# yuw444/fastF

Measured on AMD Instinct MI355X. Metric: BAM records/sec -> deduped UMI matrix; achieved HBM GB/s vs roofline, higher is better.
Workload: dtype u64

## Files before the change

### fastf_amd/csrc/umi_engine.hip

```cpp
#include "umi_kernels.hpp"
#include "sweep_kernels.hpp"

#include <algorithm>
#include <cstdarg>
#include <cstdio>
#include <cstdlib>
#include <cstring>
#include <initializer_list>
#include <mutex>
#include <new>
#include <stdexcept>
#include <chrono>
#include <string>
#include <thread>
#include <utility>
#include <vector>

extern "C" {
#include "fastf_amd.h"
#include "host_io.h"
#include "mt_jump.h"
}

using namespace fastf;
// ... 132 lines not shown
    for (size_t o = 0; o < bytes; o += HostBounce::BYTES) {
        const size_t n = std::min(bytes - o, HostBounce::BYTES);
        memcpy(g_bounce.p, (const char*)h_src + o, n);
        HIP_OK(hipMemcpyAsync((char*)d_dst + o, g_bounce.p, n, hipMemcpyHostToDevice, s));
        HIP_OK(hipStreamSynchronize(s));
    }
    return 0;
}

struct KernelTimer {
    std::vector<std::pair<hipEvent_t, hipEvent_t>> ev;
    size_t used = 0;
};

enum { AN_CAP_HITS, AN_GENE_SUMMARY, AN_GENE_MOMENTS, AN_NBR_GRAM, AN_LABEL_VOTES, AN_MARKER_AUC, AN_FAMILIES };
struct AnalysisState {
    bool attr[AN_FAMILIES] = {};
    DevBuf d_nbr;
    DevBuf d_coex;
};

enum { T_K1A, T_SCATTER, T_K3, T_COUNT, T_K1B, T_GATHER, T_TIMERS };

struct fastf_multi;
struct fastf_engine {
    fastf_multi* multi = nullptr;
    int device = 0;
    hipStream_t s_compute = nullptr, s_copy = nullptr, s_mt = nullptr;
    hipEvent_t ev_mt = nullptr;
    KeyLayout L{};
    u32 cell_bits = 0, feat_bits = 0, n_cells = 0, n_features = 0;
    u64 threshold = 0;
    u32 n_shards = 1, shard_rank = 0;
    DevBuf tab_cells, tab_feats;
    Table cells{}, feats{};
    DevBuf img_cells, img_genes;
    DevBuf d_cell_filter; MissFilter cell_filter{nullptr, 0};
    CellLds lds_cells{}; GeneLds lds_genes{};
    bool cell16 = false;
    bool use_lds_cells = false, use_lds_genes = false; u32 genes_blocks_per_cu = 1, cells_blocks_per_cu = 1;
    fastf_mt_t mt{};
    u32 mt_seed0 = 0; u64 mt_skip0 = 0;
    u64 mt_hits = 0;
    u64 mt_abs0 = 0;
    bool mt_live = false;
    DevBuf d_ring; u64 ring_len = 0;
    u32 ring_carry = 0;
    DevBuf d_dbits;
    DevBuf d_mtwords;
    bool mtwords_kept = false; u32 mtwords_seed = 0; u64 mtwords_skip = 0, mtwords_n = 0;
    AnalysisState an;
    DevBuf d_mt; bool mt_on_device = false;
    u32 mt_dev_idx = MT_N;
    bool mt_par_ready = false;
    DevBuf d_mtsub, d_mtpoly, d_mtseat, d_mtseq;
    u64 draws_up = 0;
    u64 draws_valid = 0;
    u64 batch_cap = 0;
    struct Slot {
        void* h_stage = nullptr;
        void* h_draws = nullptr;
        DevBuf d_stage;
        hipEvent_t ev_copy = nullptr, ev_done = nullptr;
        u64* h_small = nullptr;
        bool busy = false; u64 n = 0; bool external = false;
    } slot[2];
    int cur = 0;
    const u32* cur_umi_ext = nullptr;
    u64 inflight_records = 0;
    u64 key_cap = 0;
    DevBuf d_keys, d_tmp;
    DevBuf d_small;
    u64* h_small = nullptr;
    DevBuf d_feature, d_cell, d_count, d_ukeys, d_ncopy;
    u32* h_coo = nullptr; u64 h_coo_cap = 0, h_nnz = 0;
    bool h_coo_pinned = false; u32 h_coo_uses = 0;
    u32* lent_rows = nullptr; u64 lent_cap = 0;
    u32* rows_at = nullptr; u64 rows_stride = 0;
    std::vector<u32> h_ufeature, h_ucell, h_uumi, h_ncopy;
    std::vector<uint8_t> h_unonnull;
    u64 total_records = 0, hits_so_far = 0, keys_so_far = 0;
    u64 c_sampled = 0, c_valid = 0;
    bool finished = false; int sorted_in_tmp = 0; u64 n_sorted = 0;
    u32 skip_bits = 0;
    bool fully_sorted = false;
    DevBuf d_cellidx, d_tilecnt, d_tilebase, d_binbase, d_cnt;
    DevBuf d_halfhits;
    DevBuf d_segkeys;
    DevBuf d_segcount, d_segprefix, d_tileseg;
    u32 giant_parity = 0;
    u32 seg_n = 0; u64 seg_stride = 0;
    DevBuf d_rgn_phys, d_rgn_hist, d_rgn_blk;
    u32 rgn_hist_n = 0, rgn_hist_shift = 0;
    bool stream_mode = false, store_regions = false;
    bool stream_single = false, stream_sharded = false, stream_off = false;
    bool narrow = false, genes_one_family = false;
    u64 slots_used = 0, slot_cap = 0; u32 rgn_n = 0, rgn_cap = 0;
    DevBuf d_scanblk;
    u32 grid_cus = 256; int tile_grid_cap = 0; u32 k3_per_cu = 4;
    DevBuf d_rg_feature, d_rg_cell, d_rg_count, d_rg_ukeys, d_spanrows, d_spanbase, d_giant;
    u32 rg_n = 0; bool rg_umi = false;
    bool wide = false, long_umi = false; u32 group_bits = 0;
    u32 sub_bits = 0, row_split = 0;
    bool finish_queued = false;
    DevBuf d_vals, d_vtmp;
    bool timing = false;
// ... 183 lines not shown
    const u32 words = (u32)((range + 31) / 32), rank_pad = (words + 1u) & ~1u;
    size_t bytes = (((size_t)words * 4 + (size_t)rank_pad * 2 + best_n * 2) + 15) & ~(size_t)15;
    const size_t direct_bytes = ((size_t)range * 2 + 15) & ~(size_t)15;
    const bool direct = direct_bytes <= bytes + bytes / 8 && !getenv("FASTF_GENES_NO_DIRECT");
    if (direct) bytes = direct_bytes;
    {
        const char* mk = getenv("FASTF_GENES_LDS_MAX_KB");
        if (bytes > (size_t)(mk ? atoi(mk) : 152) * 1024) return 0;
    }
    std::vector<u32> img(bytes / 4 + 4, 0u);
    if (direct) {
        unsigned short* tab = reinterpret_cast<unsigned short*>(img.data());
        for (u32 i = 0; i < n; ++i) if ((keys[i] >> 44) == best) tab[(keys[i] & VM) - vmin] = (unsigned short)(i + 1);
    }
    u32* bitmap = img.data();
    unsigned short* rank = reinterpret_cast<unsigned short*>(img.data() + words);
    unsigned short* perm = rank + rank_pad;
    if (!direct) {
        std::vector<std::pair<u64, u32>> vals; vals.reserve(best_n);
        for (u32 i = 0; i < n; ++i) if ((keys[i] >> 44) == best) vals.push_back({(keys[i] & VM) - vmin, i + 1});
        std::sort(vals.begin(), vals.end());
        for (size_t r = 0; r < vals.size(); ++r) { bitmap[vals[r].first >> 5] |= 1u << (vals[r].first & 31); perm[r] = (unsigned short)vals[r].second; }
        u32 acc = 0;
        for (u32 w = 0; w < words; ++w) { rank[w] = (unsigned short)acc; acc += (u32)__builtin_popcount(bitmap[w]); }
    }
    if (e->img_genes.ensure(bytes)) return 1;
    if (copy_h2d(e->img_genes.p, img.data(), bytes)) return 1;
    e->lds_genes.image = (const u32*)e->img_genes.p; e->lds_genes.words = words; e->lds_genes.n_perm = (u32)best_n;
    e->lds_genes.family = (u32)best; e->lds_genes.vmin = vmin; e->lds_genes.range = range; e->lds_genes.bytes = (u32)bytes; e->lds_genes.direct = direct ? 1u : 0u;
    {
        for (const void* f : {(const void*)filter_pack_kernel<true, false>, (const void*)filter_pack_kernel<true, true>})
            if (hipFuncSetAttribute(f, hipFuncAttributeMaxDynamicSharedMemorySize, (int)bytes) != hipSuccess) return 0;
        for (u32 i = 0; i < N_STREAM_KERNELS; ++i)
            if (hipFuncSetAttribute((const void*)stream_kernel(i), hipFuncAttributeMaxDynamicSharedMemorySize, (int)bytes) != hipSuccess) return 0;
    }
    const size_t per_block = bytes + 1024;
    e->genes_blocks_per_cu = (u32)std::max<size_t>(1, std::min<size_t>(3, (160 * 1024) / per_block));
    e->use_lds_genes = true;
    e->genes_one_family = best_n == n;
    return 0;
}
template <size_t... I> static StreamKernel stream_kernel_of(u32 i, std::index_sequence<I...>) {
    static const StreamKernel k[] = {filter_pack_stream_kernel<(I & 4) != 0, (I & 2) != 0, (I & 1) != 0, (I >> 3) >= 1, (I >> 3) == 2>...};
    return k[i];
}
static StreamKernel stream_kernel(u32 i) { return stream_kernel_of(i, std::make_index_sequence<N_STREAM_KERNELS>{}); }

static void decide_stream_k1b(fastf_engine* e) {
    const bool can = e->use_lds_genes && !e->wide;
    e->stream_single = can && e->n_shards == 1;
    e->stream_sharded = can && e->n_shards > 1 && e->n_shards <= (u32)MAX_SHARDS;
    e->stream_off = getenv("FASTF_NO_STREAM_K1B") != nullptr;
}

extern "C" int fastf_engine_create(const fastf_engine_config_t* cfg, fastf_engine_t** out) FASTF_TRY {
    if (!cfg || !out) return set_err("null argument");
    *out = nullptr;
    const char* pf_ = getenv("FASTF_PROFILE");
    const bool lap_on = pf_ && pf_[0] == '2';
    const auto t_0 = std::chrono::steady_clock::now();
    auto lap = [&](const char* what) { if (lap_on) fprintf(stderr, "[engine create] %s at %.1f ms\n", what, std::chrono::duration<double, std::milli>(std::chrono::steady_clock::now() - t_0).count()); };
    int ndev = 0;
    hipError_t he = hipGetDeviceCount(&ndev);
    lap("device count");
    if (he != hipSuccess || ndev == 0)
        return set_err("no HIP device available (%s): the engine has no CPU fallback", hipGetErrorString(he));
    if (cfg->umi_max_bases < 1 || cfg->umi_max_bases > 32) return set_err("umi_max_bases must be 1..32");
    if (cfg->n_devices > 1 || (cfg->n_devices == 1 && getenv("FASTF_FORCE_MULTI"))) {
        fastf_engine* me = new fastf_engine();
        if (multi_create(cfg, me)) { multi_destroy(me); delete me; return 1; }
        *out = me;
        return 0;
    }
    if (cfg->device < 0 || cfg->device >= ndev) return set_err("device %d out of range (have %d)", cfg->device, ndev);
    if (cfg->n_shards < 1 || cfg->n_shards > 8 || cfg->shard_rank >= cfg->n_shards) return set_err("bad shard config");
    HIP_OK(hipSetDevice(cfg->device));
    { hipDeviceProp_t pr; if (hipGetDeviceProperties(&pr, cfg->device) == hipSuccess && pr.multiProcessorCount > 0) g_cu_count = (u32)pr.multiProcessorCount; }
    lap("device set, properties");

    fastf_engine* e = new fastf_engine();
    e->device = cfg->device;
    {
        e->grid_cus = g_cu_count;
        const char* gc = getenv("FASTF_GRID_CUS");
        if (gc) e->grid_cus = (u32)std::min<long>(std::max<long>(atol(gc), 1), (long)g_cu_count);
        const char* tc = getenv("FASTF_TILE_GRID_CAP");
        e->tile_grid_cap = tc ? std::max(atoi(tc), 8) : 0;
        const char* kc = getenv("FASTF_K3_PER_CU");
        e->k3_per_cu = kc ? (u32)std::max(atoi(kc), 1) : 4u;
    }
    e->n_cells = cfg->n_cells; e->n_features = cfg->n_features;
    e->cell16 = cfg->n_cells <= 65535u && !getenv("FASTF_CELL_SCRATCH_32");
    e->cell_bits = bits_for(cfg->n_cells);
    e->feat_bits = bits_for(cfg->n_features);
    e->L.umi_bits = 2 * cfg->umi_max_bases;
    e->L.umi_max_bytes = (cfg->umi_max_bases + 3) / 4;
    e->L.len_bits = bits_for(e->L.umi_max_bytes);
    if (cfg->umi_max_bases > 24) {
        e->sub_bits = WIDE_SUB_BITS; e->L.umi_max_bytes = 8; e->L.len_bits = WIDE_SUB_LEN_BITS; e->L.umi_bits = WIDE_SUB_VAL_BITS - WIDE_SUB_LEN_BITS;
    }
    e->L.feat_shift = 1 + e->L.umi_bits + e->L.len_bits;
    e->L.cell_shift = e->L.feat_shift + e->feat_bits;
    e->L.total_bits = e->L.cell_shift + e->cell_bits;
    e->wide = e->L.total_bits > 64 || cfg->umi_max_bases > 16 || getenv("FASTF_FORCE_WIDE_KEYS") != nullptr;
    e->long_umi = cfg->umi_max_bases > 16;
    e->group_bits = e->cell_bits + e->feat_bits + e->sub_bits;
// ... 7 lines not shown
        const char* sk = getenv("FASTF_SORT_SKIP_BITS");
        const u32 fs = e->L.feat_shift, kb = e->L.total_bits;
        const u32 passes = (kb - fs + 7) / 8;
        e->skip_bits = sk ? (u32)atoi(sk) : (kb > 8 * passes ? kb - 8 * passes : 0);
        if (e->skip_bits >= fs) e->skip_bits = 0;
        if (e->wide) e->skip_bits = 0;
    }
    e->n_shards = cfg->n_shards; e->shard_rank = cfg->shard_rank;
    e->mt_seed0 = cfg->mt_seed; e->mt_skip0 = cfg->mt_skip;

    int rc = 0;
    do {
        int prio_lo = 0, prio_hi = 0;
        const char* sp = getenv("FASTF_STREAM_PRIORITY");
        const bool high = sp && sp[0] == '1' && hipDeviceGetStreamPriorityRange(&prio_lo, &prio_hi) == hipSuccess && prio_hi != prio_lo;
        auto mk = [&](hipStream_t* s) { return high ? hipStreamCreateWithPriority(s, hipStreamNonBlocking, prio_hi) : hipStreamCreateWithFlags(s, hipStreamNonBlocking); };
        if (mk(&e->s_compute) != hipSuccess ||
            mk(&e->s_copy) != hipSuccess ||
            mk(&e->s_mt) != hipSuccess ||
            hipEventCreateWithFlags(&e->ev_mt, hipEventDisableTiming) != hipSuccess ||
            hipEventCreateWithFlags(&e->slot[0].ev_copy, hipEventDisableTiming) != hipSuccess ||
            hipEventCreateWithFlags(&e->slot[1].ev_copy, hipEventDisableTiming) != hipSuccess ||
            hipEventCreateWithFlags(&e->slot[0].ev_done, hipEventDisableTiming) != hipSuccess ||
            hipEventCreateWithFlags(&e->slot[1].ev_done, hipEventDisableTiming) != hipSuccess ||
            hipEventCreate(&e->t_ev[0]) != hipSuccess || hipEventCreate(&e->t_ev[1]) != hipSuccess) {
            rc = set_err("stream/event creation failed"); break;
        }
        lap("streams and events");
        if ((rc = build_table((const u64*)cfg->cell_keys, cfg->n_cells, e->tab_cells, e->cells, "cell"))) break;
        if ((rc = build_table((const u64*)cfg->feature_keys, cfg->n_features, e->tab_feats, e->feats, "feature"))) break;
        {
            const char* lt = getenv("FASTF_LDS_TABLES");
            if (!(lt && lt[0] == '0')) {
                const char* lc = getenv("FASTF_LDS_CELLS");
                if (!(lc && lc[0] == '0') && (rc = build_cell_lds(e, (const u64*)cfg->cell_keys, cfg->n_cells))) break;
                if (!e->use_lds_cells && (rc = build_cell_filter(e, (const u64*)cfg->cell_keys, cfg->n_cells))) break;
                if ((rc = build_gene_lds(e, (const u64*)cfg->feature_keys, cfg->n_features))) break;
            }
        }
        lap("tables built and uploaded");
        if ((rc = e->d_small.ensure(SM_WORDS * sizeof(u64)))) break;
        if (hipHostMalloc((void**)&e->h_small, SM_WORDS * sizeof(u64), hipHostMallocDefault) != hipSuccess) {
            rc = set_err("hipHostMalloc failed"); break;
        }
        if (hipMemset(e->d_small.p, 0, SM_WORDS * sizeof(u64)) != hipSuccess) { rc = set_err("memset failed"); break; }
        lap("counters allocated and cleared");
        if (set_scatter_lds_limit()) {
            rc = set_err("cannot raise dynamic LDS limit to %zu bytes", scatter_smem_bytes()); break;
        }
        lap("kernel attributes (code object loaded)");
        e->batch_cap = cfg->batch_records ? cfg->batch_records : (4ull << 20);
        e->key_cap = cfg->key_capacity;
        decide_stream_k1b(e);
        e->stream_mode = e->stream_single && !e->stream_off && !getenv("FASTF_PUSH_TILE_FORM");
        {
            const char* bw = getenv("FASTF_BLOCK_WIDE");
            e->narrow = e->stream_mode && e->genes_one_family && e->lds_genes.vmin + e->lds_genes.range <= 0xFFFFFFFFull &&
                        e->L.umi_bits <= 24 && !(bw && bw[0] == '1');
        }
    } while (0);
    if (rc) { fastf_engine_destroy(e); return 1; }
    *out = e;
    return 0;
} FASTF_CATCH_INT

extern "C" void fastf_engine_destroy(fastf_engine_t* e) FASTF_TRY {
    if (!e) return;
    if (e->multi) { multi_destroy(e); delete e; return; }
    (void)hipSetDevice(e->device);
    (void)hipDeviceSynchronize();
    for (int i = 0; i < 2; ++i) {
        fastf_engine::Slot& sl = e->slot[i];
        if (sl.h_stage) (void)hipHostFree(sl.h_stage);
        if (sl.h_draws) (void)hipHostFree(sl.h_draws);
        if (sl.h_small) (void)hipHostFree(sl.h_small);
        sl.d_stage.release();
        if (sl.ev_copy) (void)hipEventDestroy(sl.ev_copy);
        if (sl.ev_done) (void)hipEventDestroy(sl.ev_done);
        if (e->t_ev[i]) (void)hipEventDestroy(e->t_ev[i]);
    }
    if (e->h_small) (void)hipHostFree(e->h_small);
    if (e->h_coo) { if (e->h_coo_pinned) pin_unreg(e->h_coo); fastf_big_free(e->h_coo, (size_t)e->h_coo_cap * 12); }
    e->d_ring.release(); e->d_mt.release(); e->an.d_nbr.release(); e->an.d_coex.release(); e->d_dbits.release(); e->d_mtwords.release(); e->d_mtsub.release(); e->d_mtpoly.release(); e->d_mtseat.release(); e->d_mtseq.release();
    DevBuf* all[] = {&e->tab_cells, &e->tab_feats, &e->img_cells, &e->img_genes, &e->d_cell_filter, &e->d_keys, &e->d_tmp, &e->d_small, &e->d_feature, &e->d_cell,
                     &e->d_count, &e->d_ukeys, &e->d_ncopy, &e->d_cellidx, &e->d_tilecnt, &e->d_tilebase, &e->d_binbase, &e->d_cnt, &e->d_rg_feature, &e->d_rg_cell, &e->d_rg_count, &e->d_rg_ukeys, &e->d_spanrows, &e->d_spanbase, &e->d_giant, &e->d_scanblk,
                     &e->d_halfhits, &e->d_segcount, &e->d_segprefix, &e->d_tileseg, &e->d_segkeys, &e->d_vals, &e->d_vtmp,
                     &e->d_rgn_phys, &e->d_rgn_hist, &e->d_rgn_blk};
    for (DevBuf* b : all) b->release();
    if (e->s_compute) (void)hipStreamDestroy(e->s_compute);
    if (e->s_copy) (void)hipStreamDestroy(e->s_copy);
    if (e->s_mt) (void)hipStreamDestroy(e->s_mt);
    if (e->ev_mt) (void)hipEventDestroy(e->ev_mt);
    delete e;
} FASTF_CATCH_VOID

extern "C" int fastf_engine_table_modes(const fastf_engine_t* e, int* cells_in_lds, int* genes_in_lds) FASTF_TRY {
    if (!e) return set_err("null engine");
    if (cells_in_lds) *cells_in_lds = e->use_lds_cells;
    if (genes_in_lds) *genes_in_lds = e->use_lds_genes ? (e->lds_genes.direct ? 2 : 1) : 0;
    return 0;
} FASTF_CATCH_INT

extern "C" int fastf_engine_cell_scratch_bytes(const fastf_engine_t* e, uint32_t* bytes) FASTF_TRY {
    if (!e || !bytes) return set_err("null argument");
    *bytes = (e->multi ? e->n_cells <= 65535u : e->cell16) ? 2u : 4u;
    return 0;
// ... 160 lines not shown
static void launch_block_records(const fastf_engine* e, const u64* gx, const u32* umi, const u32* meta, u64 n, void* blk, hipStream_t s) {
    const u64 units = (n + BLK_RECS - 1) / BLK_RECS;
    const dim3 grid(block_records_grid(e, units));
    if (e->narrow) hipLaunchKernelGGL(block_records_kernel<true>, grid, dim3(256), 0, s, gx, umi, meta, n, (unsigned char*)blk,
                                      blk_run_bytes(e->cell16, true), e->lds_genes.family, e->L);
    else hipLaunchKernelGGL(block_records_kernel<false>, grid, dim3(256), 0, s, gx, umi, meta, n, (unsigned char*)blk,
                            blk_run_bytes(e->cell16, false), 0u, e->L);
}

extern "C" int fastf_dev_block_records(fastf_engine_t* e, const uint64_t* d_gx_key, const uint32_t* d_umi, const uint32_t* d_meta,
                                       uint64_t n, void* d_blocked, void* stream) FASTF_TRY {
    DEV_ENTRY(!e || !d_blocked, "null argument");
    if (n == 0) return 0;
    launch_block_records(e, (const u64*)d_gx_key, d_umi, d_meta, n, d_blocked, (hipStream_t)stream);
    HIP_OK(hipGetLastError());
    dbg_sync((hipStream_t)stream, "block_records");
    return 0;
} FASTF_CATCH_INT

extern "C" int fastf_dev_count_hits_blocked(fastf_engine_t* e, const uint64_t* d_cb_key, uint64_t n, void* d_blocked,
                                            uint64_t* d_hits_out, void* stream) FASTF_TRY {
    DEV_ENTRY(!e || !d_blocked, "null argument");
    hipStream_t s = (hipStream_t)stream;
    if (n == 0) { HIP_OK(hipMemsetAsync(d_hits_out, 0, sizeof(u64), s)); return 0; }
    return launch_probe_cells(e, (const u64*)d_cb_key, n, (u64*)d_hits_out, s, nullptr, nullptr, d_blocked);
} FASTF_CATCH_INT

static int launch_draw_bits(u32 cus, u64 threshold, const u32* d_draws, u64 n, u32* d_bits, hipStream_t s, u64 first = 0, u64 ring_mask = ~0ull) {
    if (n == 0) return 0;
    const u32 grid = draw_bits_grid(cus, n);
    hipLaunchKernelGGL(draw_bits_kernel, dim3(grid), dim3(256), 0, s, d_draws, n, threshold, d_bits, first, ring_mask);
    HIP_OK(hipGetLastError());
    return 0;
}
struct PlaneOut { const u64* thresholds; u32 n; u64* planes; u64 stride; };
static int launch_draw_planes(u32 cus, const PlaneOut& po, const u32* d_draws, u64 n, hipStream_t s) {
    if (n == 0) return 0;
    const u32 grid = draw_bits_grid(cus, n);
    for (u32 j0 = 0; j0 < po.n; j0 += PLANES_MAX) {
        PlaneSet ps{}; ps.n = std::min<u32>(PLANES_MAX, po.n - j0);
        for (u32 j = 0; j < ps.n; ++j) ps.threshold[j] = po.thresholds[j0 + j];
        hipLaunchKernelGGL(draw_planes_kernel, dim3(grid), dim3(256), 0, s, d_draws, n, ps, po.planes + (u64)j0 * po.stride, po.stride);
    }
    HIP_OK(hipGetLastError());
    return 0;
}
static int launch_mt_decisions(u32 cus, hipStream_t s, u32* d_mt, DevBuf& words, u32* d_ring, u64 first, u64 count, u64 ring_mask, u64 threshold, const PlaneOut* po = nullptr,
                               bool words_only = false) {
    if (count == 0) return 0;
    if (words.bytes < count * 4) {
        if (words.p) HIP_OK(hipStreamSynchronize(s));
        if (words.ensure(std::max<u64>(count * 4, 1u << 20))) return 1;
    }
    hipLaunchKernelGGL(mt_fill_kernel, dim3(1), dim3(256), 0, s, d_mt, (u32*)words.p, 0ull, count, ~0ull);
    HIP_OK(hipGetLastError());
    if (words_only) return 0;
    if (po) return launch_draw_planes(cus, *po, (const u32*)words.p, count, s);
    return launch_draw_bits(cus, threshold, (const u32*)words.p, count, d_ring, s, first, ring_mask);
}
static u32 mt_idx_after(u32 idx, u64 n) {
    if (n == 0) return idx;
    if (idx + n <= MT_N) return (u32)(idx + n);
    return (u32)((idx + n - 1) % MT_N) + 1u;
}
constexpr u64 MT_PAR_MIN = 4ull * MT_SUB_DRAWS;
static int launch_mt_decisions_par(fastf_engine* e, hipStream_t s, u32* d_mt, u32* idx, DevBuf& words, u32* d_ring, u64 first, u64 count,
                                   u64 ring_mask, u64 threshold, const PlaneOut* po = nullptr, bool words_only = false) {
    if (count == 0) return 0;
    e->mtwords_kept = false;
    static const bool no_par = getenv("FASTF_MT_SERIAL") != nullptr;
    const u64 head = *idx < MT_N ? std::min<u64>(count, MT_N - *idx) : 0;
    if (count < MT_PAR_MIN || no_par) {
        if (launch_mt_decisions(e->grid_cus, s, d_mt, words, d_ring, first, count, ring_mask, threshold, po, words_only)) return 1;
        *idx = mt_idx_after(*idx, count);
        return 0;
    }
    if (words.bytes < count * 4) {
        if (words.p) HIP_OK(hipStreamSynchronize(s));
        if (words.ensure(std::max<u64>(count * 4, 1u << 20))) return 1;
    }
    if (!e->mt_par_ready) {
        static_assert(MT_POLY_WORDS == FASTF_MT_POLY_WORDS && MT_SUB_DRAWS == FASTF_MT_SUB_DRAWS && MT_JUMP_R == FASTF_MT_JUMP_R, "kernel and table agree");
        if (e->d_mtpoly.ensure((size_t)FASTF_MT_JUMP_POLYS * MT_POLY_WORDS * sizeof(u64))) return 1;
        if (copy_h2d(e->d_mtpoly.p, fastf_mt_jump_table(), (size_t)FASTF_MT_JUMP_POLYS * MT_POLY_WORDS * sizeof(u64))) return 1;
        HIP_OK(hipFuncSetAttribute((const void*)mt_seq_kernel, hipFuncAttributeMaxDynamicSharedMemorySize, (int)(MT_SEQ_WORDS * sizeof(u32))));
        HIP_OK(hipFuncSetAttribute((const void*)mt_conv_kernel, hipFuncAttributeMaxDynamicSharedMemorySize, (int)(MT_CONV_LDS_WORDS * sizeof(u32))));
        if (e->d_mtseq.ensure((size_t)MT_JUMP_R * MT_SEQ_STRIDE * sizeof(u32))) return 1;
        e->mt_par_ready = true;
    }
    u32* const w = (u32*)words.p;
    if (head) {
        hipLaunchKernelGGL(mt_fill_kernel, dim3(1), dim3(256), 0, s, d_mt, w, 0ull, head, ~0ull);
    }
    constexpr u64 ROUND_DRAWS = (u64)MT_JUMP_R * MT_JUMP_R * MT_SUB_DRAWS;
    u64 at = head, last = 0;
    while (at < count) {
        const u64 body = std::min<u64>(count - at, ROUND_DRAWS);
        const u32 S = (u32)((body + MT_SUB_DRAWS - 1) / MT_SUB_DRAWS);
        if (e->d_mtsub.bytes < (size_t)S * MT_STATE_WORDS * 4) {
            if (e->d_mtsub.p) HIP_OK(hipStreamSynchronize(s));
            if (e->d_mtsub.ensure((size_t)std::max<u32>(S, 64) * MT_STATE_WORDS * 4)) return 1;
        }
        u32* const sub = (u32*)e->d_mtsub.p;
        u32* const seq = (u32*)e->d_mtseq.p;
        HIP_OK(hipMemcpyAsync(sub, d_mt, MT_STATE_WORDS * 4, hipMemcpyDeviceToDevice, s));
        if (S > 1) HIP_OK(hipMemsetAsync(sub + MT_STATE_WORDS, 0, (size_t)(S - 1) * MT_STATE_WORDS * 4, s));
        const u32 n_coarse = (S + MT_JUMP_R - 1) / MT_JUMP_R;
        if (n_coarse > 1) {
            hipLaunchKernelGGL(mt_seq_kernel, dim3(1), dim3(256), MT_SEQ_WORDS * sizeof(u32), s, (const u32*)sub, seq, 1u, S);
            hipLaunchKernelGGL(mt_conv_kernel, dim3(2 * (n_coarse - 1)), dim3(512), MT_CONV_LDS_WORDS * sizeof(u32), s, sub, (const u32*)seq, (const u64*)e->d_mtpoly.p, 1u, S);
        }
        if (S > 1) {
            hipLaunchKernelGGL(mt_seq_kernel, dim3(n_coarse), dim3(256), MT_SEQ_WORDS * sizeof(u32), s, (const u32*)sub, seq, MT_JUMP_R, S);
            hipLaunchKernelGGL(mt_conv_kernel, dim3(2 * n_coarse * (MT_JUMP_R - 1)), dim3(512), MT_CONV_LDS_WORDS * sizeof(u32), s, sub, (const u32*)seq, (const u64*)e->d_mtpoly.p, 0u, S);
        }
        hipLaunchKernelGGL(mt_fill_multi_kernel, dim3(S), dim3(256), 0, s, sub, w + at, 0ull, body, ~0ull);
        HIP_OK(hipMemcpyAsync(d_mt, sub + (size_t)(S - 1) * MT_STATE_WORDS, MT_STATE_WORDS * 4, hipMemcpyDeviceToDevice, s));
        HIP_OK(hipGetLastError());
        last = body - (u64)(S - 1) * MT_SUB_DRAWS;
        at += body;
    }
    *idx = mt_idx_after(MT_N, last);
    if (words_only) return 0;
    if (po) return launch_draw_planes(e->grid_cus, *po, (const u32*)w, count, s);
    return launch_draw_bits(e->grid_cus, threshold, (const u32*)w, count, d_ring, s, first, ring_mask);
}

extern "C" int fastf_dev_mt_decisions(fastf_engine_t* e, uint32_t seed, uint64_t skip, uint64_t n_draws, uint32_t* d_bits_out, void* stream) FASTF_TRY {
    DEV_ENTRY(!e || (n_draws && !d_bits_out), "null argument");
    fastf_mt_t mt; fastf_mt_seed(&mt, seed); fastf_mt_skip(&mt, skip);
    if (e->d_mtseat.ensure(sizeof mt)) return 1;
    if (copy_h2d_on(e->d_mtseat.p, &mt, sizeof mt, (hipStream_t)stream)) return 1;
    u32 idx = (u32)mt.idx;
    if (launch_mt_decisions_par(e, (hipStream_t)stream, (u32*)e->d_mtseat.p, &idx, e->d_mtwords, d_bits_out, 0, n_draws, ~0ull, e->threshold)) return 1;
    if (hipStreamSynchronize((hipStream_t)stream) != hipSuccess) return set_err("the generator kernels failed: %s", hipGetErrorString(hipGetLastError()));
    return 0;
} FASTF_CATCH_INT

extern "C" int fastf_dev_mt_decisions_multi(fastf_engine_t* e, uint32_t seed, uint64_t skip, uint64_t n_draws, const uint64_t* thresholds,
                                            uint32_t n_thresholds, uint32_t* d_planes_out, uint64_t plane_stride_words, void* stream) FASTF_TRY {
    DEV_SINGLE(!e || (n_thresholds && !thresholds) || (n_draws && n_thresholds && !d_planes_out), "null argument");
    if (n_draws && n_thresholds && ((plane_stride_words & 1) || plane_stride_words < (n_draws + 63) / 64 * 2 || ((uintptr_t)d_planes_out & 7)))
        return set_err("fastf_dev_mt_decisions_multi: planes are 8-byte aligned and an even number of 32-bit words apart, at least (n_draws + 63) / 64 * 2");
    for (u32 j = 0; j < n_thresholds; ++j)
        if (thresholds[j] > (1ull << 32)) return set_err("fastf_dev_mt_decisions_multi: threshold %u is above 2^32", j);
    HIP_OK(hipSetDevice(e->device));
    if (!n_draws || !n_thresholds) return 0;
    fastf_mt_t mt; fastf_mt_seed(&mt, seed); fastf_mt_skip(&mt, skip);
    if (e->d_mtseat.ensure(sizeof mt)) return 1;
    if (copy_h2d_on(e->d_mtseat.p, &mt, sizeof mt, (hipStream_t)stream)) return 1;
    u32 idx = (u32)mt.idx;
    const PlaneOut po{(const u64*)thresholds, n_thresholds, (u64*)d_planes_out, plane_stride_words / 2};
    if (launch_mt_decisions_par(e, (hipStream_t)stream, (u32*)e->d_mtseat.p, &idx, e->d_mtwords, nullptr, 0, n_draws, ~0ull, 0, &po)) return 1;
    if (hipStreamSynchronize((hipStream_t)stream) != hipSuccess) return set_err("the generator kernels failed: %s", hipGetErrorString(hipGetLastError()));
    return 0;
} FASTF_CATCH_INT

extern "C" void* fastf_devmem_alloc(int device, size_t bytes) FASTF_TRY {
    void* p = nullptr;
    if (hipSetDevice(device) != hipSuccess || hipMalloc(&p, bytes ? bytes : 1) != hipSuccess) {
        set_err("device allocation of %zu bytes failed: %s", bytes, hipGetErrorString(hipGetLastError()));
        return nullptr;
    }
    return p;
} FASTF_CATCH_(return nullptr)
extern "C" void fastf_devmem_free(void* p) { if (p) (void)hipFree(p); }
extern "C" int fastf_devmem_copy(void* dst, const void* src, size_t bytes) FASTF_TRY {
    if (!bytes) return 0;
    HIP_OK(hipMemcpy(dst, src, bytes, hipMemcpyDefault));
    return 0;
} FASTF_CATCH_INT
extern "C" int fastf_devmem_zero(void* dst, size_t bytes) FASTF_TRY {
    if (!bytes) return 0;
    HIP_OK(hipMemset(dst, 0, bytes));
    return 0;
} FASTF_CATCH_INT
// ... 705 lines not shown
    if (draws) {
        if (retire_all(e)) return 1;
        HIP_OK(hipStreamSynchronize(e->s_copy));
        src.ext = draws; src.ext_abs0 = e->hits_so_far; src.ext_n = n_draws;
        e->draws_up = e->hits_so_far; e->draws_valid = e->hits_so_far + n_draws;
        e->ring_carry = 0;
        e->mt_live = false; e->mt_on_device = false;
    } else if (!e->mt_live) {
        if (retire_all(e)) return 1;
        HIP_OK(hipStreamSynchronize(e->s_copy));
        fastf_mt_seed(&e->mt, e->mt_seed0);
        fastf_mt_skip(&e->mt, e->mt_skip0 + e->mt_hits);
        e->mt_abs0 = e->hits_so_far - e->mt_hits;
        e->draws_up = e->hits_so_far; e->draws_valid = e->hits_so_far;
        e->ring_carry = 0;
        e->mt_live = true;
        e->mt_on_device = false;
        if (device_mt_wanted()) {
            static_assert(sizeof(fastf_mt_t) == (MT_N + 1) * 4, "fastf_mt_t: 624 state words + the read index");
            HIP_OK(hipStreamSynchronize(e->s_mt));
            e->mtwords_kept = false;
            if (e->d_mt.ensure(sizeof(fastf_mt_t)) || e->d_mtwords.ensure(e->ring_len * 4)) return 1;
            if (copy_h2d(e->d_mt.p, &e->mt, sizeof(fastf_mt_t))) return 1;
            e->mt_dev_idx = (u32)e->mt.idx;
            e->mt_on_device = true;
        }
    }
    size_t off = 0;
    while (off < batch->n) {
        const size_t n = std::min<size_t>(batch->n - off, e->batch_cap);
        if (push_chunk(e, batch, off, n, src, pinned)) return 1;
        off += n;
    }
    if (draws) {
        if (retire_all(e)) return 1;
        HIP_OK(hipStreamSynchronize(e->s_copy));
    } else if (!pinned) {
    }
    return 0;
}

extern "C" int fastf_debug_mt_fill(int device, uint32_t seed, uint64_t skip, const uint64_t* counts, uint32_t n_calls, uint32_t* out) FASTF_TRY {
    HIP_OK(hipSetDevice(device));
    fastf_mt_t mt; fastf_mt_seed(&mt, seed); fastf_mt_skip(&mt, skip);
    u64 total = 0;
    for (u32 i = 0; i < n_calls; ++i) total += counts[i];
    DevBuf st, buf;
    int rc = 0;
    do {
        if (st.ensure(sizeof mt) || buf.ensure(std::max<u64>(total, 1) * 4)) { rc = 1; break; }
        if (copy_h2d(st.p, &mt, sizeof mt)) { rc = 1; break; }
        u64 at = 0;
        for (u32 i = 0; i < n_calls; ++i) {
            hipLaunchKernelGGL(mt_fill_kernel, dim3(1), dim3(256), 0, (hipStream_t)0, (u32*)st.p, (u32*)buf.p, at, counts[i], ~0ull);
            at += counts[i];
        }
        if (hipDeviceSynchronize() != hipSuccess || hipGetLastError() != hipSuccess) { rc = set_err("mt_fill_kernel failed"); break; }
        if (total && copy_d2h(out, buf.p, total * 4)) { rc = 1; break; }
    } while (0);
    st.release(); buf.release();
    return rc;
} FASTF_CATCH_INT

extern "C" int fastf_debug_mt_fill_bits(int device, uint32_t seed, uint64_t skip, uint64_t first, const uint64_t* counts, uint32_t n_calls,
                                        uint64_t threshold, uint64_t ring_bits, uint32_t* out) FASTF_TRY {
    if (ring_bits < 64 || (ring_bits & (ring_bits - 1))) return set_err("ring_bits must be a power of two >= 64");
    HIP_OK(hipSetDevice(device));
    fastf_mt_t mt; fastf_mt_seed(&mt, seed); fastf_mt_skip(&mt, skip);
    DevBuf st, buf, words;
    int rc = 0;
    do {
        if (st.ensure(sizeof mt) || buf.ensure(ring_bits / 8)) { rc = 1; break; }
        if (copy_h2d(st.p, &mt, sizeof mt) || hipMemset(buf.p, 0xFF, ring_bits / 8) != hipSuccess) { rc = set_err("copy failed"); break; }
        u64 at = first;
        for (u32 i = 0; i < n_calls; ++i) {
            if (launch_mt_decisions(g_cu_count, (hipStream_t)0, (u32*)st.p, words, (u32*)buf.p, at, counts[i], ring_bits - 1, threshold)) { rc = 1; break; }
            at += counts[i];
        }
        if (hipDeviceSynchronize() != hipSuccess || hipGetLastError() != hipSuccess) { rc = set_err("mt_fill_kernel failed"); break; }
        if (copy_d2h(out, buf.p, ring_bits / 8)) { rc = 1; break; }
    } while (0);
    st.release(); buf.release(); words.release();
    return rc;
} FASTF_CATCH_INT

extern "C" int fastf_engine_push(fastf_engine_t* e, const fastf_batch_t* batch) FASTF_TRY {
    return push_impl(e, batch, nullptr, 0, false);
} FASTF_CATCH_INT

extern "C" int fastf_engine_push_draws(fastf_engine_t* e, const fastf_batch_t* batch, const uint32_t* draws, size_t n_draws) FASTF_TRY {
    if (!draws && batch && batch->n) return set_err("null draws");
    return push_impl(e, batch, draws, n_draws, false);
} FASTF_CATCH_INT

extern "C" int fastf_engine_push_pinned(fastf_engine_t* e, const fastf_batch_t* batch) FASTF_TRY {
    if (batch && batch->n && (debug_known_memory(batch->cb_key, batch->n * 8, "fastf_engine_push_pinned cb_key") || debug_known_memory(batch->gx_key, batch->n * 8, "fastf_engine_push_pinned gx_key") ||
                              debug_known_memory(batch->umi, batch->n * 4, "fastf_engine_push_pinned umi") || debug_known_memory(batch->meta, batch->n * 4, "fastf_engine_push_pinned meta")))
        return 1;
    return push_impl(e, batch, nullptr, 0, true);
} FASTF_CATCH_INT

extern "C" int fastf_engine_wait_input(fastf_engine_t* e) FASTF_TRY {
    if (!e) return set_err("null engine");
    if (e->multi) return 0;
    HIP_OK(hipSetDevice(e->device));
    HIP_OK(hipStreamSynchronize(e->s_copy));
    return 0;
// ... 418 lines not shown
```

### fastf_amd/csrc/umi_kernels.hpp

```cpp
#pragma once
#if !defined(FASTF_EXPERIMENT)
#  if defined(FASTF_X_ANY)
#    error "FASTF_X_* knobs need -DFASTF_EXPERIMENT (experiment builds only: tools/build_variant.sh)"
#  endif
#endif
#ifndef FASTF_K1_IPT
#define FASTF_K1_IPT 8
#endif
#ifndef FASTF_K1_THREADS
#define FASTF_K1_THREADS 512
#endif
#include <hip/hip_runtime.h>
#include <stdint.h>
#include <type_traits>

namespace fastf {

typedef unsigned long long u64;
typedef unsigned int u32;

constexpr int WAVE = 64;

constexpr u64 ERR_DRAWS_SHORT  = 2;
constexpr u64 ERR_UMI_TOOLONG  = 4;
// ... 21 lines not shown
#ifndef FASTF_NT_SORT
#define FASTF_NT_SORT FASTF_NT_ALL
#endif
#ifndef FASTF_NT_K3
#define FASTF_NT_K3 FASTF_NT_ALL
#endif
typedef u64 u64x2_t __attribute__((ext_vector_type(2)));
template <bool NT, class T> __device__ __forceinline__ T ld_once(const T* p) {
    if constexpr (NT) return __builtin_nontemporal_load(p); else return *p;
}
template <bool NT> __device__ __forceinline__ ulonglong2 ld_once2(const u64* p) {
    if constexpr (NT) { const u64x2_t v = __builtin_nontemporal_load(reinterpret_cast<const u64x2_t*>(p)); return make_ulonglong2(v.x, v.y); }
    else return *reinterpret_cast<const ulonglong2*>(p);
}
__device__ __forceinline__ u64 wave_sum64(u64 v) {
#pragma unroll
    for (int o = 32; o > 0; o >>= 1) v += __shfl_xor(v, o, WAVE);
    return v;
}
__device__ __forceinline__ u32 wave_sum32(u32 v) {
#pragma unroll
    for (int o = 32; o > 0; o >>= 1) v += __shfl_xor(v, o, WAVE);
    return v;
}
__device__ __forceinline__ u32 wave_incl_scan32(u32 v, int lane) {
#pragma unroll
    for (int o = 1; o < WAVE; o <<= 1) {
        u32 t = __shfl_up(v, o, WAVE);
        if (lane >= o) v += t;
    }
    return v;
}
__device__ __forceinline__ u64 uniform64(u64 v) {
    return ((u64)(u32)__builtin_amdgcn_readfirstlane((int)(u32)(v >> 32)) << 32) | (u64)(u32)__builtin_amdgcn_readfirstlane((int)(u32)v);
}
__device__ __forceinline__ u64 mix64(u64 x) {
    x ^= x >> 33; x *= 0xff51afd7ed558ccdULL;
    x ^= x >> 33; x *= 0xc4ceb9fe1a85ec53ULL;
    x ^= x >> 33;
    return x;
}

__global__ void clear_bits_kernel(u64* word, u64 mask) { atomicAnd(word, ~mask); }

constexpr u32 MT_N = 624, MT_M = 397;
__device__ __forceinline__ u32 mt_mix(u32 hi, u32 lo) {
    const u32 y = (hi & 0x80000000u) | (lo & 0x7fffffffu);
    return (y >> 1) ^ ((0u - (y & 1u)) & 0x9908b0dfu);
}
__device__ __forceinline__ u32 mt_temper(u32 y) {
    y ^= y >> 11; y ^= (y << 7) & 0x9d2c5680u; y ^= (y << 15) & 0xefc60000u; y ^= y >> 18;
    return y;
}
__device__ __forceinline__ void mt_fill_body(u32 (&buf)[2][MT_N], u32* __restrict__ state, u32* __restrict__ out, u64 first, u64 count, u64 mask) {
    const u32 tid = threadIdx.x;
    for (u32 i = tid; i < MT_N; i += 256) buf[0][i] = state[i];
    u32 idx = state[MT_N];
    u32 cur = 0;
    __syncthreads();
    u64 done = 0;
    if (idx < MT_N && count) {
        const u32 take = (u32)(count < (u64)(MT_N - idx) ? count : (u64)(MT_N - idx));
        for (u32 i = tid; i < take; i += 256) out[(first + i) & mask] = mt_temper(buf[0][idx + i]);
        idx += take; done = take;
    }
    while (done < count) {
        const u32* o = buf[cur]; u32* n = buf[cur ^ 1];
        const u64 left = count - done;
        const u64 at = first + done;
        if (tid < MT_N - MT_M) { const u32 v = o[tid + MT_M] ^ mt_mix(o[tid], o[tid + 1]); n[tid] = v; if (tid < left) out[(at + tid) & mask] = mt_temper(v); }
        __syncthreads();
        const u32 k2 = tid + (MT_N - MT_M);
        if (tid < MT_N - MT_M) { const u32 v = n[k2 - (MT_N - MT_M)] ^ mt_mix(o[k2], o[k2 + 1]); n[k2] = v; if (k2 < left) out[(at + k2) & mask] = mt_temper(v); }
        __syncthreads();
        const u32 k3 = tid + 2 * (MT_N - MT_M);
        if (k3 < MT_N) {
            const u32 v = k3 < MT_N - 1 ? n[k3 - (MT_N - MT_M)] ^ mt_mix(o[k3], o[k3 + 1]) : n[MT_M - 1] ^ mt_mix(o[MT_N - 1], n[0]);
            n[k3] = v;
            if (k3 < left) out[(at + k3) & mask] = mt_temper(v);
        }
        __syncthreads();
        cur ^= 1;
        idx = (u32)(left < (u64)MT_N ? left : (u64)MT_N);
        done += idx;
    }
    for (u32 i = tid; i < MT_N; i += 256) state[i] = buf[cur][i];
    if (tid == 0) state[MT_N] = idx;
}
__global__ __launch_bounds__(256) void mt_fill_kernel(u32* __restrict__ state, u32* __restrict__ out, u64 first, u64 count, u64 mask) {
    __shared__ u32 buf[2][MT_N];
    mt_fill_body(buf, state, out, first, count, mask);
}

constexpr u32 MT_SUB_DRAWS = 624u * 256u, MT_POLY_WORDS = 312, MT_DEG = 19937, MT_STATE_WORDS = MT_N + 1;
constexpr u32 MT_JUMP_SWEEPS = 88, MT_SEQ_WORDS = MT_N + MT_JUMP_SWEEPS * (MT_N - MT_M);
static_assert(MT_SEQ_WORDS >= MT_N + MT_DEG + 16, "the sequence covers the windows of every coefficient (and the sixteen outputs beyond 624 a lane reads along)");
constexpr u32 MT_SEQ_STRIDE = 20736;
constexpr u32 MT_JUMP_R = 32;
constexpr u32 MT_HALF_PW = MT_POLY_WORDS / 2, MT_HALF_X = MT_HALF_PW * 64u + 640u, MT_CONV_WAVES = 8;
constexpr u32 MT_CONV_LDS_WORDS = MT_HALF_X + 16u + MT_CONV_WAVES * 640u;
static_assert(MT_POLY_WORDS % 2 == 0 && MT_HALF_PW * 64u + MT_HALF_X <= MT_SEQ_STRIDE, "a half's bulk load stays inside its sequence's stride");
__global__ __launch_bounds__(256) void mt_seq_kernel(const u32* __restrict__ states, u32* __restrict__ seq, u32 src_stride, u32 n_sub) {
    extern __shared__ __attribute__((aligned(16))) unsigned char mtj_smem[];
    u32* const X = reinterpret_cast<u32*>(mtj_smem);
    const u32 src = blockIdx.x * src_stride;
    if (src >= n_sub) return;
    const u32 tid = threadIdx.x;
    const u32* const a = states + (u64)src * MT_STATE_WORDS;
    for (u32 i = tid; i < MT_N; i += 256) X[i] = a[i];
    __syncthreads();
    for (u32 sw = 0; sw < MT_JUMP_SWEEPS; ++sw) {
        if (tid < MT_N - MT_M) { const u32 t = sw * (MT_N - MT_M) + tid; X[t + MT_N] = X[t + MT_M] ^ mt_mix(X[t], X[t + 1]); }
        __syncthreads();
    }
    u32* const out = seq + (u64)blockIdx.x * MT_SEQ_STRIDE;
    for (u32 i = tid; i < MT_SEQ_WORDS; i += 256) out[i] = X[i];
}
__device__ __forceinline__ u64 lds_read_u64_alone(const u64* p) {
    typedef __attribute__((address_space(3))) const u64 lds_u64;
    u32 a = (u32)(uintptr_t)(lds_u64*)p;
    asm volatile("" : "+v"(a));
    return *(lds_u64*)(uintptr_t)a;
}
__global__ __launch_bounds__(512, 2) void mt_conv_kernel(u32* __restrict__ states, const u32* __restrict__ seq, const u64* __restrict__ polys, u32 coarse, u32 n_sub) {
    extern __shared__ __attribute__((aligned(16))) unsigned char mtj_smem[];
    u32* const X = reinterpret_cast<u32*>(mtj_smem);
    const u32 job = blockIdx.x >> 1, half = blockIdx.x & 1u;
    const u32 c = coarse ? 0u : job / (MT_JUMP_R - 1u), i = coarse ? job + 1u : job % (MT_JUMP_R - 1u) + 1u;
    const u32 dst = coarse ? i * MT_JUMP_R : c * MT_JUMP_R + i;
    if (dst >= n_sub) return;
    const u64* const poly = polys + (u64)((coarse ? MT_JUMP_R - 1u : 0u) + i - 1u) * MT_POLY_WORDS + (u64)half * MT_HALF_PW;
    const u32 tid = threadIdx.x;
    {
        const uint4* const g = reinterpret_cast<const uint4*>(seq + (u64)c * MT_SEQ_STRIDE + (u64)half * MT_HALF_PW * 64u);
        uint4* const l = reinterpret_cast<uint4*>(X);
        for (u32 q = tid; q < MT_HALF_X / 4u; q += 512) l[q] = g[q];
    }
    __syncthreads();
    u32* const part = X + MT_HALF_X + 16u;
    {
        const u32 lane = tid & 63u, w = tid >> 6;
        u64 ae[5], ao[5];
#pragma unroll
        for (int q = 0; q < 5; ++q) { ae[q] = 0; ao[q] = 0; }
// ... 3 lines not shown
            const u32 hi = __builtin_amdgcn_bitop3_b32((u32)(a >> 32), (u32)(b >> 32), (u32)(c >> 32), 0x96);
            return (u64)lo | ((u64)hi << 32);
        };
        auto walk = [&](u64 bits, const u64* const base, u64 (&acc)[5]) {
            while (bits) {
                const u32 n = (u32)__builtin_popcountll(bits);
                if (n >= 4) {
                    const u32 k0 = (u32)__builtin_ctzll(bits); bits &= bits - 1;
                    const u32 k1 = (u32)__builtin_ctzll(bits); bits &= bits - 1;
                    const u32 k2 = (u32)__builtin_ctzll(bits); bits &= bits - 1;
                    const u32 k3 = (u32)__builtin_ctzll(bits); bits &= bits - 1;
                    const u64 *x0 = base + (k0 >> 1), *x1 = base + (k1 >> 1), *x2 = base + (k2 >> 1), *x3 = base + (k3 >> 1);
                    u64 t0[5], t1[5], t2[5], t3[5];
#pragma unroll
                    for (int q = 0; q < 5; ++q) {
                        t0[q] = lds_read_u64_alone(x0 + 64 * q); t1[q] = lds_read_u64_alone(x1 + 64 * q);
                        t2[q] = lds_read_u64_alone(x2 + 64 * q); t3[q] = lds_read_u64_alone(x3 + 64 * q);
                    }
#pragma unroll
                    for (int q = 0; q < 5; ++q) acc[q] = xor3(xor3(acc[q], t0[q], t1[q]), t2[q], t3[q]);
                } else {
                    const u32 k0 = (u32)__builtin_ctzll(bits); bits &= bits - 1;
                    const u64* const x0 = base + (k0 >> 1);
#pragma unroll
                    for (int q = 0; q < 5; ++q) acc[q] ^= x0[64 * q];
                }
            }
        };
        for (u32 pw = w; pw < MT_HALF_PW; pw += MT_CONV_WAVES) {
            const u64 bits = uniform64(poly[pw]);
            const u64* const base = X64 + (pw << 5) + lane;
            walk(bits & 0x5555555555555555ull, base, ae);
            walk(bits & 0xAAAAAAAAAAAAAAAAull, base, ao);
        }
        u32 carry = 0;
#pragma unroll
        for (int q = 4; q >= 0; --q) {
            const u32 o_lo = (u32)ao[q];
            const u32 from_above = (u32)__builtin_amdgcn_update_dpp((int)carry, (int)o_lo, 0x130, 0xF, 0xF, false);
            carry = (u32)__builtin_amdgcn_readlane((int)o_lo, 0);
            const u32 v_lo = (u32)ae[q] ^ (u32)(ao[q] >> 32), v_hi = (u32)(ae[q] >> 32) ^ from_above;
            *reinterpret_cast<u64*>(part + w * 640u + 2u * (lane + 64u * q)) = (u64)v_lo | ((u64)v_hi << 32);
        }
    }
    __syncthreads();
    for (u32 t = tid; t < MT_N; t += 512) {
        u32 v = 0;
#pragma unroll
        for (u32 w = 0; w < MT_CONV_WAVES; ++w) v ^= part[w * 640u + t];
        if (v) atomicXor(&states[(u64)dst * MT_STATE_WORDS + t], v);
    }
    if (tid == 0 && half == 0) states[(u64)dst * MT_STATE_WORDS + MT_N] = MT_N;
}
__global__ __launch_bounds__(256) void mt_fill_multi_kernel(u32* __restrict__ states, u32* __restrict__ out, u64 first, u64 count, u64 mask) {
    __shared__ u32 buf[2][MT_N];
    const u64 off = (u64)blockIdx.x * MT_SUB_DRAWS;
    if (off >= count) return;
    const u64 n = count - off < (u64)MT_SUB_DRAWS ? count - off : (u64)MT_SUB_DRAWS;
    mt_fill_body(buf, states + (u64)blockIdx.x * MT_STATE_WORDS, out, first + off, n, mask);
}

__global__ __launch_bounds__(256) void draw_bits_kernel(const u32* __restrict__ draws, u64 n, u64 threshold, u32* __restrict__ bits, u64 first, u64 ring_mask) {
    const int lane = lane_id();
    u64* const bits64 = reinterpret_cast<u64*>(bits);
    const u64 wmask = ring_mask >> 6, w_first = first >> 6, end = first + n;
    const u64 n_words = n ? ((end + 63) >> 6) - w_first : 0;
    const u64 waves = (u64)gridDim.x * (256 / WAVE), w0 = (u64)blockIdx.x * (256 / WAVE) + (threadIdx.x >> 6);
    constexpr u32 U = 4;
    for (u64 c0 = w0 * U; c0 < n_words; c0 += waves * U) {
        u32 d[U]; bool in[U];
#pragma unroll
        for (u32 u = 0; u < U; ++u) {
            const u64 r = ((w_first + c0 + u) << 6) + (u64)lane;
            in[u] = c0 + u < n_words && r >= first && r < end;
            d[u] = draws[in[u] ? r - first : 0];
        }
#pragma unroll
        for (u32 u = 0; u < U; ++u) {
            const u64 c = c0 + u;
            const u64 m = __ballot(in[u] && (u64)d[u] < threshold);
            if (lane == 0 && c < n_words) {
                u64* const w = bits64 + ((w_first + c) & wmask);
                const u32 low = c == 0 ? (u32)(first & 63u) : 0u;
                *w = low ? (*w & ((1ull << low) - 1ull)) | m : m;
            }
        }
    }
}

struct Table { const uint4* slots; u32 mask; };

__device__ __forceinline__ u32 slot_hash(u64 key) {
    const u32 h = (u32)key * 0x9E3779B1u + (u32)(key >> 32) * 0x85EBCA77u;
    return h ^ (h >> 15);
}

__device__ __forceinline__ u32 table_probe(const Table t, u64 key) {
    if (key == 0) return 0;
    u32 h = slot_hash(key) & t.mask;
    for (u32 i = 0; i <= t.mask; ++i) {
        const uint4 s = t.slots[h];
        const u64 k = ((u64)s.y << 32) | s.x;
        if (k == key) return s.z;
        if (k == 0) return 0;
        h = (h + 1) & t.mask;
    }
    return 0;
}

struct KeyLayout {
    u32 umi_bits;
    u32 len_bits;
// ... 1987 lines not shown
```

Before: 108.1 billion.

## Fuse Mersenne Twister fill with threshold bit packing in parallel decision path

The parallel MT decision path can now temper each generated draw, compare it against the threshold and ballot the results straight into the bit ring inside the fill kernels. This replaces the separate write of 32-bit draw words followed by a draw_bits pass. Word boundaries that straddle sub-streams are handled by having the tail block generate a few draws ahead into the following block's range. The fused path runs only when there is no ring wrap, no planes and a 64-aligned start, and an environment variable disables it. It adds index arithmetic and extra LDS reads inside the serial MT loop.

```diff
diff --git a/fastf_amd/csrc/umi_engine.hip b/fastf_amd/csrc/umi_engine.hip
--- a/fastf_amd/csrc/umi_engine.hip
+++ b/fastf_amd/csrc/umi_engine.hip
@@ -208,6 +208,7 @@
     AnalysisState an;
     DevBuf d_mt; bool mt_on_device = false;
     u32 mt_dev_idx = MT_N;
+    bool mt_fused_off = false;
     bool mt_par_ready = false;
     DevBuf d_mtsub, d_mtpoly, d_mtseat, d_mtseq;
     u64 draws_up = 0;
@@ -497,6 +498,7 @@
     e->stream_sharded = can && e->n_shards > 1 && e->n_shards <= (u32)MAX_SHARDS;
     e->stream_off = getenv("FASTF_NO_STREAM_K1B") != nullptr;
 }
+static void decide_mt_fused(fastf_engine* e) { e->mt_fused_off = getenv("FASTF_NO_FUSED_DECISIONS") != nullptr; }
 
 extern "C" int fastf_engine_create(const fastf_engine_config_t* cfg, fastf_engine_t** out) FASTF_TRY {
     if (!cfg || !out) return set_err("null argument");
@@ -610,6 +612,7 @@
         e->batch_cap = cfg->batch_records ? cfg->batch_records : (4ull << 20);
         e->key_cap = cfg->key_capacity;
         decide_stream_k1b(e);
+        decide_mt_fused(e);
         e->stream_mode = e->stream_single && !e->stream_off && !getenv("FASTF_PUSH_TILE_FORM");
         {
             const char* bw = getenv("FASTF_BLOCK_WIDE");
@@ -876,7 +879,7 @@
         if (words.p) HIP_OK(hipStreamSynchronize(s));
         if (words.ensure(std::max<u64>(count * 4, 1u << 20))) return 1;
     }
-    hipLaunchKernelGGL(mt_fill_kernel, dim3(1), dim3(256), 0, s, d_mt, (u32*)words.p, 0ull, count, ~0ull);
+    hipLaunchKernelGGL(mt_fill_kernel<false>, dim3(1), dim3(256), 0, s, d_mt, (u32*)words.p, 0ull, count, ~0ull, 0ull, 0ull);
     HIP_OK(hipGetLastError());
     if (words_only) return 0;
     if (po) return launch_draw_planes(cus, *po, (const u32*)words.p, count, s);
@@ -899,7 +902,8 @@
         *idx = mt_idx_after(*idx, count);
         return 0;
     }
-    if (words.bytes < count * 4) {
+    const bool fused = !e->mt_fused_off && !po && !words_only && ring_mask == ~0ull && (first & 63u) == 0;
+    if (!fused && words.bytes < count * 4) {
         if (words.p) HIP_OK(hipStreamSynchronize(s));
         if (words.ensure(std::max<u64>(count * 4, 1u << 20))) return 1;
     }
@@ -914,7 +918,8 @@
     }
     u32* const w = (u32*)words.p;
     if (head) {
-        hipLaunchKernelGGL(mt_fill_kernel, dim3(1), dim3(256), 0, s, d_mt, w, 0ull, head, ~0ull);
+        if (fused) hipLaunchKernelGGL(mt_fill_kernel<true>, dim3(1), dim3(256), 0, s, d_mt, d_ring, first, head, ~0ull, threshold, count - head);
+        else hipLaunchKernelGGL(mt_fill_kernel<false>, dim3(1), dim3(256), 0, s, d_mt, w, 0ull, head, ~0ull, 0ull, 0ull);
     }
     constexpr u64 ROUND_DRAWS = (u64)MT_JUMP_R * MT_JUMP_R * MT_SUB_DRAWS;
     u64 at = head, last = 0;
@@ -938,14 +943,15 @@
             hipLaunchKernelGGL(mt_seq_kernel, dim3(n_coarse), dim3(256), MT_SEQ_WORDS * sizeof(u32), s, (const u32*)sub, seq, MT_JUMP_R, S);
             hipLaunchKernelGGL(mt_conv_kernel, dim3(2 * n_coarse * (MT_JUMP_R - 1)), dim3(512), MT_CONV_LDS_WORDS * sizeof(u32), s, sub, (const u32*)seq, (const u64*)e->d_mtpoly.p, 0u, S);
         }
-        hipLaunchKernelGGL(mt_fill_multi_kernel, dim3(S), dim3(256), 0, s, sub, w + at, 0ull, body, ~0ull);
+        if (fused) hipLaunchKernelGGL(mt_fill_multi_kernel<true>, dim3(S), dim3(256), 0, s, sub, d_ring, first + at, body, ~0ull, threshold, count - at - body);
+        else hipLaunchKernelGGL(mt_fill_multi_kernel<false>, dim3(S), dim3(256), 0, s, sub, w + at, 0ull, body, ~0ull, 0ull, 0ull);
         HIP_OK(hipMemcpyAsync(d_mt, sub + (size_t)(S - 1) * MT_STATE_WORDS, MT_STATE_WORDS * 4, hipMemcpyDeviceToDevice, s));
         HIP_OK(hipGetLastError());
         last = body - (u64)(S - 1) * MT_SUB_DRAWS;
         at += body;
     }
     *idx = mt_idx_after(MT_N, last);
-    if (words_only) return 0;
+    if (words_only || fused) return 0;
     if (po) return launch_draw_planes(e->grid_cus, *po, (const u32*)w, count, s);
     return launch_draw_bits(e->grid_cus, threshold, (const u32*)w, count, d_ring, s, first, ring_mask);
 }
@@ -1757,7 +1763,7 @@
         if (copy_h2d(st.p, &mt, sizeof mt)) { rc = 1; break; }
         u64 at = 0;
         for (u32 i = 0; i < n_calls; ++i) {
-            hipLaunchKernelGGL(mt_fill_kernel, dim3(1), dim3(256), 0, (hipStream_t)0, (u32*)st.p, (u32*)buf.p, at, counts[i], ~0ull);
+            hipLaunchKernelGGL(mt_fill_kernel<false>, dim3(1), dim3(256), 0, (hipStream_t)0, (u32*)st.p, (u32*)buf.p, at, counts[i], ~0ull, 0ull, 0ull);
             at += counts[i];
         }
         if (hipDeviceSynchronize() != hipSuccess || hipGetLastError() != hipSuccess) { rc = set_err("mt_fill_kernel failed"); break; }
diff --git a/fastf_amd/csrc/umi_kernels.hpp b/fastf_amd/csrc/umi_kernels.hpp
--- a/fastf_amd/csrc/umi_kernels.hpp
+++ b/fastf_amd/csrc/umi_kernels.hpp
@@ -97,44 +97,92 @@
     y ^= y >> 11; y ^= (y << 7) & 0x9d2c5680u; y ^= (y << 15) & 0xefc60000u; y ^= y >> 18;
     return y;
 }
-__device__ __forceinline__ void mt_fill_body(u32 (&buf)[2][MT_N], u32* __restrict__ state, u32* __restrict__ out, u64 first, u64 count, u64 mask) {
+template <bool BITS>
+__device__ __forceinline__ void mt_fill_body(u32 (&buf)[2][MT_N], u32* __restrict__ state, u32* __restrict__ out, u64 first, u64 count, u64 mask,
+                                             u64 threshold = 0, u64 after = 0) {
     const u32 tid = threadIdx.x;
     for (u32 i = tid; i < MT_N; i += 256) buf[0][i] = state[i];
     u32 idx = state[MT_N];
     u32 cur = 0;
     __syncthreads();
     u64 done = 0;
+    const u32 lane = tid & 63u, wv = tid >> 6;
+    u64* const bits64 = reinterpret_cast<u64*>(out);
+    long long base = -(long long)idx;
+    u64 wnext = (0 - first) & 63u;
+    const u32* const flat = &buf[0][0];
+    auto word_of = [&](int r) -> u32 {
+        const int a = (int)(cur * MT_N) + r;
+        return (u32)(a + ((a >> 31) & (int)(2 * MT_N)));
+    };
+    u32 ev[3], e_nw = 0;
+    u64* e_to = nullptr;
+    auto emit_load = [&](u64 E) {
+        e_nw = E >= wnext + 64 ? (u32)((E - wnext) >> 6) : 0u;
+        const int r0 = (int)((long long)wnext - base) + (int)tid;
+        const u32 a0 = word_of(r0);
+        e_to = bits64 + ((first + wnext) >> 6) + wv;
+#pragma unroll
+        for (u32 u = 0; u < 3; ++u) { const u32 a = u ? cur * MT_N + (u32)r0 + 256u * u : a0; ev[u] = flat[a < 2 * MT_N ? a : 0u]; }
+    };
+    auto emit_store = [&]() {
+#pragma unroll
+        for (u32 u = 0; u < 3; ++u) {
+            const u64 m = __ballot((u64)mt_temper(ev[u]) < threshold);
+            if (lane == 0 && wv + 4u * u < e_nw) e_to[4u * u] = m;
+        }
+        wnext += 64ull * e_nw;
+    };
     if (idx < MT_N && count) {
         const u32 take = (u32)(count < (u64)(MT_N - idx) ? count : (u64)(MT_N - idx));
-        for (u32 i = tid; i < take; i += 256) out[(first + i) & mask] = mt_temper(buf[0][idx + i]);
+        if constexpr (!BITS) for (u32 i = tid; i < take; i += 256) out[(first + i) & mask] = mt_temper(buf[0][idx + i]);
         idx += take; done = take;
     }
     while (done < count) {
         const u32* o = buf[cur]; u32* n = buf[cur ^ 1];
         const u64 left = count - done;
         const u64 at = first + done;
-        if (tid < MT_N - MT_M) { const u32 v = o[tid + MT_M] ^ mt_mix(o[tid], o[tid + 1]); n[tid] = v; if (tid < left) out[(at + tid) & mask] = mt_temper(v); }
+        if constexpr (BITS) emit_load(done);
+        if (tid < MT_N - MT_M) { const u32 v = o[tid + MT_M] ^ mt_mix(o[tid], o[tid + 1]); n[tid] = v; if constexpr (!BITS) if (tid < left) out[(at + tid) & mask] = mt_temper(v); }
+        if constexpr (BITS) emit_store();
         __syncthreads();
         const u32 k2 = tid + (MT_N - MT_M);
-        if (tid < MT_N - MT_M) { const u32 v = n[k2 - (MT_N - MT_M)] ^ mt_mix(o[k2], o[k2 + 1]); n[k2] = v; if (k2 < left) out[(at + k2) & mask] = mt_temper(v); }
+        if (tid < MT_N - MT_M) { const u32 v = n[k2 - (MT_N - MT_M)] ^ mt_mix(o[k2], o[k2 + 1]); n[k2] = v; if constexpr (!BITS) if (k2 < left) out[(at + k2) & mask] = mt_temper(v); }
         __syncthreads();
         const u32 k3 = tid + 2 * (MT_N - MT_M);
         if (k3 < MT_N) {
             const u32 v = k3 < MT_N - 1 ? n[k3 - (MT_N - MT_M)] ^ mt_mix(o[k3], o[k3 + 1]) : n[MT_M - 1] ^ mt_mix(o[MT_N - 1], n[0]);
             n[k3] = v;
-            if (k3 < left) out[(at + k3) & mask] = mt_temper(v);
+            if constexpr (!BITS) if (k3 < left) out[(at + k3) & mask] = mt_temper(v);
         }
         __syncthreads();
         cur ^= 1;
+        base += MT_N;
         idx = (u32)(left < (u64)MT_N ? left : (u64)MT_N);
         done += idx;
     }
+    if constexpr (BITS) {
+        emit_load(count); emit_store();
+        if (wnext < count && wv == 0) {
+            const u64 d = wnext + lane;
+            const u32* const c = buf[cur];
+            bool keep = false;
+            if (d < count) keep = (u64)mt_temper(flat[word_of((int)((long long)d - base))]) < threshold;
+            else if (d - count < after) {
+                const u32 t = (u32)(d - count);
+                keep = (u64)mt_temper(c[t + MT_M] ^ mt_mix(c[t], c[t + 1])) < threshold;
+            }
+            const u64 m = __ballot(keep);
+            if (lane == 0) bits64[(first + wnext) >> 6] = m;
+        }
+    }
     for (u32 i = tid; i < MT_N; i += 256) state[i] = buf[cur][i];
     if (tid == 0) state[MT_N] = idx;
 }
-__global__ __launch_bounds__(256) void mt_fill_kernel(u32* __restrict__ state, u32* __restrict__ out, u64 first, u64 count, u64 mask) {
+template <bool BITS>
+__global__ __launch_bounds__(256) void mt_fill_kernel(u32* __restrict__ state, u32* __restrict__ out, u64 first, u64 count, u64 mask, u64 threshold, u64 after) {
     __shared__ u32 buf[2][MT_N];
-    mt_fill_body(buf, state, out, first, count, mask);
+    mt_fill_body<BITS>(buf, state, out, first, count, mask, threshold, after);
 }
 
 constexpr u32 MT_SUB_DRAWS = 624u * 256u, MT_POLY_WORDS = 312, MT_DEG = 19937, MT_STATE_WORDS = MT_N + 1;
@@ -244,12 +292,13 @@
     }
     if (tid == 0 && half == 0) states[(u64)dst * MT_STATE_WORDS + MT_N] = MT_N;
 }
-__global__ __launch_bounds__(256) void mt_fill_multi_kernel(u32* __restrict__ states, u32* __restrict__ out, u64 first, u64 count, u64 mask) {
+template <bool BITS>
+__global__ __launch_bounds__(256) void mt_fill_multi_kernel(u32* __restrict__ states, u32* __restrict__ out, u64 first, u64 count, u64 mask, u64 threshold, u64 after) {
     __shared__ u32 buf[2][MT_N];
     const u64 off = (u64)blockIdx.x * MT_SUB_DRAWS;
     if (off >= count) return;
     const u64 n = count - off < (u64)MT_SUB_DRAWS ? count - off : (u64)MT_SUB_DRAWS;
-    mt_fill_body(buf, states + (u64)blockIdx.x * MT_STATE_WORDS, out, first + off, n, mask);
+    mt_fill_body<BITS>(buf, states + (u64)blockIdx.x * MT_STATE_WORDS, out, first + off, n, mask, threshold, count - off - n + after);
 }
 
 __global__ __launch_bounds__(256) void draw_bits_kernel(const u32* __restrict__ draws, u64 n, u64 threshold, u32* __restrict__ bits, u64 first, u64 ring_mask) {
```

Result: no change. 108.3 billion (median of 6 runs) (+0.2%).
